# SeanChenxy/TDRN

Measured on AMD Instinct MI355X. Metric: frames/sec/GPU @320x320 dualrefinedet_vggbn; box Linf vs CPU ref, higher is better.
Workload: dtype bf16; 1 GPU; dualrefinedet_vggbn 320x320 multihead, bf16, batch 32 per GPU, forward + Detect(top_k 200, conf 0.01, nms 0.45), synthetic VOC-shaped frames + synthetic weights; global_batch=32, parallelism=frame-sharded x1, no per-frame collective, launch=eager, resident_batches=4, steps_in_flight=2

## Files before the change

include/tdrn_hip.h:

```cpp
#ifndef TDRN_HIP_H
#define TDRN_HIP_H

#include <stddef.h>
#include <stdint.h>

#ifdef __cplusplus
extern "C" {
#endif

#define TDRN_API __attribute__((visibility("default")))

#define TDRN_OK 0
#define TDRN_E_ARG (-1)
#define TDRN_E_SHAPE (-2)
#define TDRN_E_WORKSPACE (-3)
#define TDRN_E_UNSUPPORTED (-4)
#define TDRN_E_PARAM (-5)
#define TDRN_E_STATE (-6)
#define TDRN_E_VALUE (-7)
#define TDRN_E_DEVICE (-8)

TDRN_API const char *tdrn_version(void);
TDRN_API const char *tdrn_error_string(int code);

// ... 233 lines not shown
                         int32_t *counts_out, void *workspace, size_t workspace_bytes,
                         void *stream);
TDRN_API int tdrn_detect_dev_scale(const float *loc, const float *conf, const float *priors,
                                   const float *arm_loc, const float *scale_dev, int B, int P, int C,
                                   int top_k, float conf_thresh, double nms_thresh, float *out,
                                   int32_t *counts_out, void *workspace, size_t workspace_bytes,
                                   void *stream);

TDRN_API int tdrn_preprocess(const uint8_t *frames, int B, int H0, int W0, int S, const float mean_bgr[3],
                             int to_rgb, float *out, void *stream);
TDRN_API int tdrn_preprocess_u8(const uint8_t *frames, int B, int H0, int W0, int S, int to_rgb, uint8_t *out, void *stream);

typedef enum {
    TDRN_DRN_VGGBN = 0,
    TDRN_DRN_MOBILENET = 1,
    TDRN_SSD4SCALE_MOBILE = 2,
    TDRN_REFINEDET_VGG = 3,
    TDRN_SSD4SCALE_VGG = 4
} tdrn_model;

typedef struct {
    int model;
    int size;
    int num_classes;
    int c7_channel;
    int def_groups;
    int bn;
    int multihead;
    int deform;
    int test_phase;
    int dtype;
    int use_refine;
    int plan_flags;
    int reserved[4];
} tdrn_net_config;

#define TDRN_PLAN_NO_FUSE_FIRST 1
#define TDRN_PLAN_NO_LATE_SIDE  2
#define TDRN_PLAN_ONE_STREAM    4
#define TDRN_PLAN_NO_DEFORM_TS  8
#define TDRN_PLAN_CHAIN         16
#define TDRN_PLAN_NO_CONV_PP    32
#define TDRN_PLAN_NO_PP_SK      64
#define TDRN_PLAN_NO_CONV_PATCH 128
#define TDRN_PLAN_DWPW          512
#define TDRN_PLAN_NO_PW1X1      1024
#define TDRN_PLAN_NO_DW_SLIDE   2048
#define TDRN_PLAN_DW_SLIDE_ALL  4096
#define TDRN_PLAN_NO_CONV_WS    8192
#define TDRN_PLAN_NO_YGEMM_V2  16384
#define TDRN_PLAN_NO_HEAD3X3   32768
#define TDRN_PLAN_TS_ONE_RANGE  65536
#define TDRN_PLAN_NO_PATCH_TAIL 131072
#define TDRN_PLAN_FAULT_HANDOFF 256

typedef struct tdrn_net tdrn_net;

TDRN_API int tdrn_net_create(const tdrn_net_config *cfg, tdrn_net **out);
TDRN_API void tdrn_net_destroy(tdrn_net *net);

TDRN_API int tdrn_net_param_count(const tdrn_net *net);
TDRN_API int tdrn_net_param_info(const tdrn_net *net, int index, const char **name,
                                 int64_t shape[4], int *ndim);
TDRN_API int tdrn_net_set_param(tdrn_net *net, const char *name, const float *data_host,
                                int64_t numel);

TDRN_API size_t tdrn_net_weight_bytes(const tdrn_net *net);
TDRN_API size_t tdrn_net_workspace_bytes(const tdrn_net *net, int batch);
TDRN_API int tdrn_net_num_priors(const tdrn_net *net);

TDRN_API int tdrn_net_pack_weights(tdrn_net *net, void *weights_dev, size_t weights_bytes,
                                   void *stream);
TDRN_API int tdrn_net_adopt_weights(tdrn_net *net);

typedef struct {
    const float *x;
    int batch;
    float *arm_loc;
    float *odm_loc;
    float *conf;
    float *offsets[4];
    const float *ref_loc[4];
    float *loc_maps[4];
    void *reserved[4];
} tdrn_net_io;
typedef struct {
    const uint8_t *planes;
    float mean[3];
} tdrn_u8_frames;

TDRN_API int tdrn_net_forward(tdrn_net *net, const void *weights_dev, void *workspace,
                              size_t workspace_bytes, const tdrn_net_io *io, void *stream);

TDRN_API int tdrn_net_check(tdrn_net *net, unsigned *detail);

typedef struct {
    char name[48];
    int launches;
    double flops;
    double bytes;
    double ms;
} tdrn_kernel_stat;
TDRN_API int tdrn_net_profile(tdrn_net *net, int enable);
TDRN_API int tdrn_net_kernel_stats(tdrn_net *net, tdrn_kernel_stat *out, int max_entries);
TDRN_API int tdrn_net_op_stats(tdrn_net *net, tdrn_kernel_stat *out, int max_entries);
TDRN_API int tdrn_net_op_timeline(tdrn_net *net, float *start_ms, float *end_ms, int *lane, int max_entries);
// ... 34 lines not shown
```

tdrn_amd/_lib.py:

```python
import ctypes as C
import os

_HERE = os.path.dirname(os.path.abspath(__file__))
LIB_PATH = os.environ.get("TDRN_LIB_PATH") or os.path.join(_HERE, "lib", "libtdrn_hip.so")

F32, BF16, F16 = 0, 1, 2
DTYPES = {"fp32": F32, "f32": F32, "float32": F32, "bf16": BF16, "bfloat16": BF16, "fp16": F16,
          "f16": F16, "float16": F16, "half": F16}
DRN_VGGBN, DRN_MOBILENET, SSD4SCALE_MOBILE, REFINEDET_VGG, SSD4SCALE_VGG = range(5)

E_VALUE = -7


class TdrnError(RuntimeError):
    def __init__(self, code, what=""):
        self.code = code
        super().__init__("%s (tdrn error %d)%s" % (error_string(code), code,
                                                    (": " + what) if what else ""))


class NetConfig(C.Structure):
    _fields_ = [("model", C.c_int), ("size", C.c_int), ("num_classes", C.c_int),
                ("c7_channel", C.c_int), ("def_groups", C.c_int), ("bn", C.c_int),
                ("multihead", C.c_int), ("deform", C.c_int), ("test_phase", C.c_int),
                ("dtype", C.c_int), ("use_refine", C.c_int), ("plan_flags", C.c_int), ("reserved", C.c_int * 4)]


PLAN_NO_FUSE_FIRST, PLAN_NO_LATE_SIDE, PLAN_ONE_STREAM, PLAN_NO_DEFORM_TS, PLAN_CHAIN = 1, 2, 4, 8, 16
PLAN_NO_CONV_PP, PLAN_NO_PP_SK, PLAN_NO_CONV_PATCH, PLAN_FAULT_HANDOFF, PLAN_DWPW, PLAN_NO_PW1X1 = 32, 64, 128, 256, 512, 1024
PLAN_NO_DW_SLIDE, PLAN_DW_SLIDE_ALL, PLAN_NO_CONV_WS, PLAN_NO_YGEMM_V2, PLAN_NO_HEAD3X3, PLAN_TS_ONE_RANGE = 2048, 4096, 8192, 16384, 32768, 65536
PLAN_NO_PATCH_TAIL = 131072
E_DEVICE = -8


class NetIO(C.Structure):
    _fields_ = [("x", C.c_void_p), ("batch", C.c_int), ("arm_loc", C.c_void_p),
                ("odm_loc", C.c_void_p), ("conf", C.c_void_p), ("offsets", C.c_void_p * 4),
                ("ref_loc", C.c_void_p * 4), ("loc_maps", C.c_void_p * 4),
                ("reserved", C.c_void_p * 4)]


class KernelStat(C.Structure):
    _fields_ = [("name", C.c_char * 48), ("launches", C.c_int), ("flops", C.c_double),
                ("bytes", C.c_double), ("ms", C.c_double)]


class U8FramesABI(C.Structure):
    _fields_ = [("planes", C.c_void_p), ("mean", C.c_float * 3)]


class OpInfo(C.Structure):
    _fields_ = [("kind", C.c_int), ("in_", C.c_int), ("out", C.c_int), ("res", C.c_int), ("pool", C.c_int), ("off", C.c_int),
                ("y", C.c_int), ("k", C.c_int), ("stride", C.c_int), ("pad", C.c_int), ("dil", C.c_int), ("relu", C.c_int),
                ("ceil_mode", C.c_int), ("splitk", C.c_int), ("groups", C.c_int), ("out_kind", C.c_int), ("level", C.c_int),
                ("n_branches", C.c_int), ("k2", C.c_int), ("pad2", C.c_int), ("off_c0", C.c_int * 2), ("y_tap_major", C.c_int),
                ("fused_first", C.c_int), ("fused_dw", C.c_int), ("w", C.c_char * 48), ("b", C.c_char * 48), ("bn", C.c_char * 48), ("w2", C.c_char * 48),
                ("b2", C.c_char * 48), ("y_groups", C.c_int)]


class AugmentParams(C.Structure):
    _fields_ = [("brightness", C.c_float), ("contrast_pre", C.c_float), ("contrast_post", C.c_float), ("saturation", C.c_float),
                ("hue", C.c_float), ("perm", C.c_int32 * 3), ("canvas_w", C.c_int32), ("canvas_h", C.c_int32),
                ("img_x", C.c_int32), ("img_y", C.c_int32), ("crop_x0", C.c_int32), ("crop_y0", C.c_int32),
                ("crop_x1", C.c_int32), ("crop_y1", C.c_int32), ("cropped", C.c_int32), ("mirror", C.c_int32),
                ("kept", C.c_int32), ("status", C.c_int32)]


class AugmentImage(C.Structure):
    _fields_ = [("data", C.c_void_p), ("h", C.c_int32), ("w", C.c_int32)]


class AugmentPairParams(C.Structure):
    _fields_ = [("base", AugmentParams), ("shift_x", C.c_double), ("shift_y", C.c_double), ("trans_x", C.c_int32),
                ("trans_y", C.c_int32), ("attempts", C.c_int32), ("reserved", C.c_int32)]


class SgdTensor(C.Structure):
    _fields_ = [("param", C.c_void_p), ("grad", C.c_void_p), ("momentum_buf", C.c_void_p), ("numel", C.c_int64),
                ("group", C.c_int32), ("reserved", C.c_int32)]


SGD_ZERO_GRADS, SGD_CHUNK, SGD_TENSORS_PER_LAUNCH = 1, 4096, 96
AUGMENT_MAX_TRUTHS, AUGMENT_MAX_SIZE = 512, 2048
AUGMENT_CROP_FALLBACK, AUGMENT_TAPE_EXHAUSTED, AUGMENT_TRANS_FALLBACK = 1, 2, 4
# ... 159 lines not shown
```

tdrn_amd/csrc/conv3x3_patch.hip:

```cpp
#include <cstdio>
#include <cstdlib>
#include <type_traits>

#include "kernels.h"
#include "mfma_prims.h"

#ifndef TDRN_PATCH_PRIO
#define TDRN_PATCH_PRIO 4
#endif
#ifndef TDRN_PATCH_ABLATE
#define TDRN_PATCH_ABLATE 0
#endif

namespace tdrn {

struct PatchParams {
    const char *in, *w, *zero;
    const float *bias;
    char *out, *out_pool;
    int B, H, W, Cin, Cout, Cs, Ktot;
    int relu;
    int tw, lgtw;
    int tiles_x, tiles_per_img;
    int m_tiles, n_tiles, items;
    int M;
    int tail_split;
    const float *fx, *fw, *fb;
    int fS, fCout;
    int ablate;
#ifdef TDRN_PATCH_STAMP
    unsigned *stamps;
#endif
#ifdef TDRN_PATCH_WGTIME
    unsigned long long *wgt;
#endif
};

#ifdef TDRN_PATCH_STAMP
#define STAMP_DECL unsigned long long st_t = __builtin_amdgcn_s_memtime(); unsigned st_acc[8] = {0, 0, 0, 0, 0, 0, 0, 0};
#define STAMP(k) do { const unsigned long long t_ = __builtin_amdgcn_s_memtime(); st_acc[k] += (unsigned)(t_ - st_t); st_t = t_; } while (0)
#define STAMP_FLUSH do { if (lane == 0) for (int k_ = 0; k_ < 8; ++k_) p.stamps[((size_t)blockIdx.x * 12 + wave) * 8 + k_] = st_acc[k_]; } while (0)
#else
#define STAMP_DECL
#define STAMP(k) do { } while (0)
#define STAMP_FLUSH do { } while (0)
#endif

namespace {

#ifndef TDRN_PATCH_RING
#define TDRN_PATCH_RING 3
#endif
constexpr int kRing = TDRN_PATCH_RING;
constexpr int kPatchSlots = kRing == 4 ? 43 : 44;
constexpr int kSlotsPerLoader = (kPatchSlots + 3) / 4;

}

template <typename DT, int BN, int TW, bool FUSE = false>
__global__ __launch_bounds__(768) void conv3x3_patch_kernel(const PatchParams p)
{
    static_assert(!FUSE || (BN == 64 && TW == 32 && sizeof(DT) == 2), "fused first conv: 16-bit, 64 couts, 8x32 tiles");
    constexpr bool FLAT = TW == 0;
    constexpr int LGTW = TW == 32 ? 5 : 4;
    constexpr int TPX = FUSE ? 512 : 256;
    constexpr int TH = TW ? TPX / TW : 0;
    constexpr int PXG = TPX / 64;
    constexpr int CG = 8 / PXG;
    constexpr int ES = elem_traits<DT>::bytes;
    constexpr int P16 = elem_traits<DT>::per16;
    constexpr int CK = 128 / ES;
    constexpr int BNH = BN / CG;
    constexpr int WC = BNH / 32;
    constexpr int WBYTES = BN * 128;
    constexpr int WL = BN / 32;
    constexpr int RING = BN == 128 ? kRing : 3;
    constexpr int SROWS = (ES == 2 ? 16 : 8) / ((RING == 4 && BN == 128) ? 2 : 1);
    constexpr int SSTRIDE = BNH * ES + 16;
    constexpr int NPB = FUSE ? 1 : 2;
    constexpr int PSLOTS = FUSE ? ((TH + 2) * (TW + 2) + 7) / 8 : kPatchSlots;
    constexpr int PBYTES = PSLOTS * 1024;
    constexpr int OFF_W = NPB * PBYTES;
    constexpr int OFF_S = OFF_W + RING * WBYTES;
    constexpr int OFF_B = OFF_S + 8 * SROWS * SSTRIDE;
    constexpr int RAWR = TH + 4, RAWC = 36;
    constexpr int RAWN = 3 * RAWR * RAWC;
    constexpr int RAWP = (RAWN + 63) / 64, RAWJ = (RAWP + 3) / 4;
    constexpr int FTILES = ((TH + 2) * (TW + 2) + 31) / 32, FTJ = (FTILES + 3) / 4;
    constexpr int RAWB = ((RAWN + 63) / 64) * 256;
    constexpr int OFF_R = OFF_B + 1024;
    constexpr int LDS = FUSE ? OFF_R + 2 * RAWB + 256 : OFF_B + 1024;
    static_assert(LDS <= 160 * 1024, "LDS budget");
    __shared__ __attribute__((aligned(16))) char smem[LDS];

    const int lane = threadIdx.x & 63;
    const int wave = __builtin_amdgcn_readfirstlane(threadIdx.x >> 6);
    const int nchunks = p.Cin / CK;
#ifdef TDRN_PATCH_WGTIME
    if (threadIdx.x == 0) p.wgt[2 * blockIdx.x] = __builtin_amdgcn_s_memrealtime();
#endif

    const XcdItems xi = xcd_items(p.items);
    const int slot = xi.slot, istride = xi.istride;
    int avail = p.items - xi.xcd * xi.per_xcd;
    avail = avail < xi.per_xcd ? avail : xi.per_xcd;
    int n_full = avail > slot ? (avail - slot + istride - 1) / istride : 0;
    const int item0 = xi.item0();
    [[maybe_unused]] int n_tail = 0, tail_enc = 0;
    constexpr bool TAILOK = BN == 128 && sizeof(DT) == 2 && !FUSE;
    if constexpr (TAILOK) {
        if (p.tail_split && avail > 0) {
            const int full = avail / istride, rem = avail - full * istride;
            if (full > 0 && rem > 0 && 2 * rem <= istride) {
                n_full = full;
                if (slot < 2 * rem) {
                    n_tail = 1;
                    tail_enc = 2 * (xi.xcd * xi.per_xcd + full * istride) + slot;
                }
            }
        }
    }
    const int n_it = n_full + n_tail;
    const int n_steps = n_it * nchunks * 9;
    auto item_mt = [&](int it) { return (it < n_full ? item0 + it * istride : tail_enc >> 1) / p.n_tiles; };
    auto item_c0 = [&](int it) {
        const int item = it < n_full ? item0 + it * istride : tail_enc >> 1;
        return (item % p.n_tiles) * BN + (it < n_full ? 0 : (tail_enc & 1) * 64);
    };
    const int RS = TW ? TW + 2 : p.W;

    if (wave >= 8) {
        if (TDRN_PATCH_PRIO == 4) __builtin_amdgcn_s_setprio(2);
        if (TDRN_PATCH_PRIO == 5) __builtin_amdgcn_s_setprio(3);
        const int lw = wave - 8;
        const int lrow = lane >> 3, pc = lane & 7;
        unsigned poff[kSlotsPerLoader];
        int pyx[kSlotsPerLoader];
// ... 164 lines not shown
                char *dst = smem + OFF_W + wslot * WBYTES;
#pragma unroll
                for (int k = 0; k < WL; ++k)
                    if (!TAILOK || k < np) lds_dma16_ptr(wfixed ? p.w + (woff[k] & 0xffffu) : wbase + wk + woff[k], dst + (lw + 4 * k) * 1024);
            }
            ++ws;
            wslot = wslot == RING - 1 ? 0 : wslot + 1;
            wk += (unsigned)(p.Cin * ES);
            if (++w_tap == 9) {
                w_tap = 0;
                if (++w_cc == nchunks) {
                    w_cc = 0;
                    ++w_it;
                    if (w_it < n_it) weight_item();
                }
                wk = (unsigned)(w_cc * 128);
            }
            return np;
        };
        auto load_patch = [&](int j, unsigned ccoff, char *dstbuf) {
            if (!live || lw + 4 * j >= kPatchSlots || FUSE) return;
            const unsigned o = poff[j];
            lds_dma16_ptr(o == 0xFFFFFFFFu ? p.zero : (pfixed ? p.in + (o & 0xfffffu) : p.in + (size_t)o + ccoff), dstbuf + (lw + 4 * j) * 1024);
        };
        int p_it = 0, p_cc = 0, pbuf = 0;
        auto next_patch_chunk = [&]() {
            if (NPB == 2) pbuf ^= 1;
            if (++p_cc == nchunks) {
                p_cc = 0;
                ++p_it;
            }
        };

        if constexpr (FUSE) {
            if (n_it > 0) load_raw(item0, 0);
            asm volatile("s_waitcnt vmcnt(0) lgkmcnt(0)" ::: "memory");
            __builtin_amdgcn_s_barrier();
            if (n_it > 0) {
                int b_;
                tile_origin(item0, b_, f_y0, f_x0);
#pragma unroll
                for (int q = 0; q < FTJ; ++q)
                    if (lw + 4 * q < FTILES) first_conv_tile(lw + 4 * q, 0, smem);
            }
        }
        if (n_it > 0) {
            weight_item();
            if constexpr (!FUSE) {
                patch_table(item_mt(0));
#pragma unroll
                for (int j = 0; j < kSlotsPerLoader; ++j) load_patch(j, 0u, smem);
            }
#pragma unroll
            for (int k = 0; k < RING - 1; ++k)
                if (k < n_steps) load_weights();
            next_patch_chunk();
            if (lw == 0 && live)
                lds_dma16_ptr(lane < (n_full > 0 ? BN : 64) / 4 ? (const char *)(p.bias + item_c0(0)) + lane * 16 : p.zero, smem + OFF_B);
        }
        asm volatile("s_waitcnt vmcnt(0) lgkmcnt(0)" ::: "memory");
        __builtin_amdgcn_s_barrier();

        int tap = 0, c_it = 0, c_cc = 0, carried = 0;
        STAMP_DECL
        const int last_piece = lw + 4 * (kSlotsPerLoader - 1) < kPatchSlots ? 1 : 0;
        for (int g = 0; g < n_steps; ++g) {
            int issued = 0;
            if (ws < n_steps) issued = load_weights();
            if constexpr (FUSE) {
                if (tap == 0 && c_it + 1 < n_it) issued += load_raw(item0 + (c_it + 1) * istride, (c_it + 1) & 1);
            } else if (p_it < n_it && tap < 6) {
                char *dstbuf = smem + pbuf * PBYTES;
                const unsigned ccoff = (unsigned)(p_cc * 128);
                switch (tap) {
                    case 0:
                        patch_table(item_mt(p_it));
                        load_patch(0, ccoff, dstbuf); load_patch(1, ccoff, dstbuf); issued += 2; break;
                    case 1: load_patch(2, ccoff, dstbuf); load_patch(3, ccoff, dstbuf); issued += 2; break;
                    case 2: load_patch(4, ccoff, dstbuf); load_patch(5, ccoff, dstbuf); issued += 2; break;
                    case 3: load_patch(6, ccoff, dstbuf); load_patch(7, ccoff, dstbuf); issued += 2; break;
                    case 4: load_patch(8, ccoff, dstbuf); load_patch(9, ccoff, dstbuf); issued += 2; break;
                    default: load_patch(10, ccoff, dstbuf); issued += last_piece; break;
                }
            }
            if (lw == 0 && c_cc == nchunks - 1 && tap == 6 && c_it + 1 < n_it) {
                if (live) lds_dma16_ptr(lane < (c_it + 1 < n_full ? BN : 64) / 4 ? (const char *)(p.bias + item_c0(c_it + 1)) + lane * 16 : p.zero, smem + OFF_B);
                issued += 1;
            }
            STAMP(0);
            wait_vmcnt(live ? issued + (RING == 4 ? carried : 0) : 0);
            if constexpr (FUSE) asm volatile("s_waitcnt lgkmcnt(0)" ::: "memory");
            STAMP(1);
            carried = issued;
            __builtin_amdgcn_s_barrier();
            STAMP(2);
            if (++tap == 9) {
                tap = 0;
                next_patch_chunk();
                if (++c_cc == nchunks) {
                    if constexpr (FUSE) {
                        if (c_it + 1 < n_it) {
                            int b_;
                            tile_origin(item0 + (c_it + 1) * istride, b_, f_y0, f_x0);
#pragma unroll
                            for (int q = 0; q < FTJ; ++q)
                                if (lw + 4 * q < FTILES) first_conv_tile(lw + 4 * q, (c_it + 1) & 1, smem);
                            asm volatile("s_waitcnt lgkmcnt(0)" ::: "memory");
                            __builtin_amdgcn_s_barrier();
                        }
                    }
                    c_cc = 0;
                    ++c_it;
                }
            }
        }
        STAMP_FLUSH;
        return;
    }

    const int r32 = lane & 31, hh = lane >> 5;
    const int cw = wave % PXG;
    const int chalf = wave / PXG;
    char *stg = smem + OFF_S + wave * SROWS * SSTRIDE;
    f32x16 acc[WC][2];

    int base_i[2];
    unsigned tapmask[2] = {0x1FFu, 0x1FFu};
    unsigned need_mask = 0;
#pragma unroll
    for (int pt = 0; pt < 2; ++pt) {
        const int i = cw * 64 + pt * 32 + r32;
        base_i[pt] = TW ? (i >> LGTW) * RS + (i & (TW - 1)) : i;
    }
    const int wsw = (r32 >> 1) & 7;
    constexpr int CPR = BNH * ES / 16;
    constexpr int RPI = 64 / CPR;
    const int my_ch = lane % CPR, my_row = lane / CPR;
    constexpr bool compute = !(TDRN_PATCH_ABLATE & 2);

    int cur_mt = -1, n0 = 0;
    long long tile_pix0 = 0;
    int tile_row0 = 0, tile_x0 = 0;
    auto setup_item = [&](int it) {
        const int mt = item_mt(it);
        n0 = item_c0(it);
        if (mt == cur_mt) return;
// ... 219 lines not shown
    int psw[2] = {(base_i[0] >> 1) & 7, (base_i[1] >> 1) & 7};
    auto load_frags = [&](auto wcn_tag, u32x4 *wf, u32x4 *pf, int kk) {
        constexpr int WCN = decltype(wcn_tag)::value;
        if (!compute) return;
        const int lc = 2 * kk + hh;
#pragma unroll
        for (int ci = 0; ci < WCN; ++ci) wf[ci] = *(const u32x4 *)(wsb + (chalf * (32 * WCN) + ci * 32 + r32) * 128 + ((lc ^ wsw) << 4));
#pragma unroll
        for (int pt = 0; pt < 2; ++pt) pf[pt] = *(const u32x4 *)(psb + prow[pt] * 128 + ((lc ^ psw[pt]) << 4));
    };
    auto mma_frags = [&](auto wcn_tag, const u32x4 *wf, u32x4 *pf, unsigned m0, unsigned m1) {
        constexpr int WCN = decltype(wcn_tag)::value;
        if (!compute) return;
        if constexpr (FLAT) {
#pragma unroll
            for (int j = 0; j < 4; ++j) {
                pf[0][j] &= m0;
                pf[1][j] &= m1;
            }
        }
#pragma unroll
        for (int ci = 0; ci < WCN; ++ci)
#pragma unroll
            for (int pt = 0; pt < 2; ++pt) Mma32<DT>::run(wf[ci], pf[pt], acc[ci][pt]);
    };
    auto init_acc = [&](auto wcn_tag) {
        constexpr int WCN = decltype(wcn_tag)::value;
        const char *bsrc = smem + OFF_B;
#pragma unroll
        for (int ci = 0; ci < WCN; ++ci)
#pragma unroll
            for (int g = 0; g < 4; ++g) {
                const f32x4 bv = *(const f32x4 *)(bsrc + (chalf * (32 * WCN) + ci * 32 + 8 * g + 4 * hh) * 4);
#pragma unroll
                for (int pt = 0; pt < 2; ++pt)
#pragma unroll
                    for (int j = 0; j < 4; ++j) acc[ci][pt][4 * g + j] = bv[j];
            }
    };

    if constexpr (FUSE) __builtin_amdgcn_s_barrier();
    __builtin_amdgcn_s_barrier();
    if (TDRN_PATCH_PRIO == 2 && wave >= 4) __builtin_amdgcn_s_setprio(1);
    if (TDRN_PATCH_PRIO == 3) __builtin_amdgcn_s_setprio(1);
    typedef std::integral_constant<int, WC> full_t;
    typedef std::integral_constant<int, 1> half_t;
    if (n_it > 0) {
        setup_item(0);
        init_acc(full_t{});
        load_frags(full_t{}, wfA, pfA, 0);
    }
    int it = 0, cc = 0, tap = 0, tq = 0, delta = 0, wslot = 0, pbuf = 0;
    STAMP_DECL
    auto step = [&](auto wcn) {
        unsigned m0 = 0xFFFFFFFFu, m1 = 0xFFFFFFFFu;
        if constexpr (FLAT) {
            m0 = ((tapmask[0] >> tap) & 1u) ? 0xFFFFFFFFu : 0u;
            m1 = ((tapmask[1] >> tap) & 1u) ? 0xFFFFFFFFu : 0u;
        }
        if (TDRN_PATCH_PRIO == 0) __builtin_amdgcn_s_setprio(1);
        load_frags(wcn, wfB, pfB, 1);
        __builtin_amdgcn_sched_barrier(0);
        mma_frags(wcn, wfA, pfA, m0, m1);
        __builtin_amdgcn_sched_barrier(0);
        load_frags(wcn, wfA, pfA, 2);
        __builtin_amdgcn_sched_barrier(0);
        mma_frags(wcn, wfB, pfB, m0, m1);
        __builtin_amdgcn_sched_barrier(0);
        load_frags(wcn, wfB, pfB, 3);
        __builtin_amdgcn_sched_barrier(0);
        mma_frags(wcn, wfA, pfA, m0, m1);
        if (TDRN_PATCH_PRIO == 0) __builtin_amdgcn_s_setprio(0);
        __builtin_amdgcn_s_waitcnt(0xC07F);
        STAMP(0);
        __builtin_amdgcn_s_barrier();
        STAMP(1);
        const bool item_done = tap == 8 && cc == nchunks - 1;
        wslot = wslot == RING - 1 ? 0 : wslot + 1;
        ++tap;
        if (++tq == 3) {
            tq = 0;
            delta += RS;
        }
        if (tap == 9) {
            tap = 0; tq = 0; delta = 0;
            pbuf ^= 1;
            if (++cc == nchunks) cc = 0;
        }
        wsb = smem + OFF_W + wslot * WBYTES;
        psb = smem + (NPB == 2 ? pbuf : 0) * PBYTES;
#pragma unroll
        for (int pt = 0; pt < 2; ++pt) {
            prow[pt] = base_i[pt] + delta + tq;
            psw[pt] = (prow[pt] >> 1) & 7;
        }
        if (!(FUSE && item_done)) load_frags(wcn, wfA, pfA, 0);
        __builtin_amdgcn_sched_barrier(0);
        if (TDRN_PATCH_PRIO == 0) __builtin_amdgcn_s_setprio(1);
        mma_frags(wcn, wfB, pfB, m0, m1);
        if (TDRN_PATCH_PRIO == 0) __builtin_amdgcn_s_setprio(0);
        STAMP(2);
        if (item_done) {
            epilogue(wcn);
            ++it;
            if (it < n_it) {
                setup_item(it);
                if (TAILOK && it >= n_full) {
                    init_acc(half_t{});
                    load_frags(half_t{}, wfA, pfA, 0);
                } else {
                    init_acc(full_t{});
                }
                if constexpr (FUSE) {
                    __builtin_amdgcn_s_barrier();
                    load_frags(wcn, wfA, pfA, 0);
                }
            }
            STAMP(3);
        }
    };
    const int n_steps_full = n_full * nchunks * 9;
#pragma unroll 1
    for (int g = 0; g < n_steps_full; ++g) step(full_t{});
    if constexpr (TAILOK) {
#pragma unroll 1
        for (int g = n_steps_full; g < n_steps; ++g) step(half_t{});
    }
    STAMP_FLUSH;
#ifdef TDRN_PATCH_WGTIME
    if (threadIdx.x == 0) p.wgt[2 * blockIdx.x + 1] = __builtin_amdgcn_s_memrealtime();
#endif
}

bool patch_takes(const ConvArgs &a, bool pooled)
{
    if ((a.kdisable & KOFF_CONV_PATCH) || a.fuse_x8 || !conv3x3_input_fits(a)) return false;
    const int mode = conv3x3_tile_mode(a, kPatchSlots);
    if (pooled && (mode < 0 || (a.H & 1) || (a.W & 1))) return false;
    if (a.fuse_x && (a.dtype == TDRN_F32 || mode != 32 || a.Npad != 64 || a.H % 16)) return false;
    return mode != 0;
}

template <typename DT, int BN> static int launch_patch_cfg(const PatchParams &p_in, hipStream_t s)
{
    PatchParams p = p_in;
    const int grid = persistent_grid(p.items);
#ifdef TDRN_PATCH_WGTIME
    static unsigned long long *wgt = nullptr;
    static long calls = 0, want = -1;
    if (!wgt) TDRN_HIP_TRY(hipMalloc((void **)&wgt, 256 * 2 * sizeof(unsigned long long)));
    if (want < 0) { const char *e = getenv("TDRN_WGTIME_CALL"); want = e ? atol(e) : 2000; }
    p.wgt = wgt;
    const bool report = calls >= want && calls < want + 18;
    ++calls;
    if (report) TDRN_HIP_TRY(hipMemsetAsync(wgt, 0, 256 * 2 * sizeof(unsigned long long), s));
    struct Report {
        bool on; hipStream_t s; int grid; const PatchParams &p; unsigned long long *d;
        ~Report() {
            if (!on) return;
            (void)hipStreamSynchronize(s);
            unsigned long long h[512];
            (void)hipMemcpy(h, d, sizeof(h), hipMemcpyDeviceToHost);
            unsigned long long t0 = ~0ull, t1 = 0;
            int n = 0;
            for (int i = 0; i < grid; ++i) if (h[2 * i]) { t0 = h[2 * i] < t0 ? h[2 * i] : t0; t1 = h[2 * i + 1] > t1 ? h[2 * i + 1] : t1; ++n; }
            double late = 0, busy = 0, worst = 0, e_min = 1e18; int n5 = 0, n20 = 0;
            for (int i = 0; i < grid; ++i) if (h[2 * i]) {
                const double d0 = (h[2 * i] - t0) * 0.01, b = (h[2 * i + 1] - h[2 * i]) * 0.01, e = (h[2 * i + 1] - t0) * 0.01;
                late += d0; busy += b; worst = d0 > worst ? d0 : worst; e_min = e < e_min ? e : e_min; n5 += d0 > 5; n20 += d0 > 20;
            }
            fprintf(stderr, "wgtime %dx%d Cin %d Cout %d items %d grid %d: span %.1f us, workgroup busy mean %.1f us, first end at %.1f us; start later than the first: mean %.1f us, max %.1f us, > 5 us: %d, > 20 us: %d of %d\n",
                    p.H, p.W, p.Cin, p.Cout, p.items, grid, (t1 - t0) * 0.01, busy / n, e_min, late / n, worst, n5, n20, n);
        }
    } rep{report, s, grid, p, wgt};
#endif
    if constexpr (BN == 64 && sizeof(DT) == 2) {
        if (p.fx) {
            hipLaunchKernelGGL((conv3x3_patch_kernel<DT, 64, 32, true>), dim3(grid), dim3(768), 0, s, p);
            return hip_status(hipGetLastError());
        }
    }
    if (p.fx) return TDRN_E_UNSUPPORTED;
    if (p.tw == 0) hipLaunchKernelGGL((conv3x3_patch_kernel<DT, BN, 0>), dim3(grid), dim3(768), 0, s, p);
    else if (p.tw == 32) hipLaunchKernelGGL((conv3x3_patch_kernel<DT, BN, 32>), dim3(grid), dim3(768), 0, s, p);
    else hipLaunchKernelGGL((conv3x3_patch_kernel<DT, BN, 16>), dim3(grid), dim3(768), 0, s, p);
    return hip_status(hipGetLastError());
}

int launch_conv3x3_patch(const ConvArgs &a, void *out_pool, hipStream_t s)
{
    if (!patch_takes(a, out_pool != nullptr)) return TDRN_E_UNSUPPORTED;
    const int mode = conv3x3_tile_mode(a, kPatchSlots);
    PatchParams p;
    p.in = (const char *)a.in; p.w = (const char *)a.w; p.zero = (const char *)a.zero_page; p.bias = a.bias;
    p.out = (char *)a.out; p.out_pool = (char *)out_pool;
    p.B = a.B; p.H = a.H; p.W = a.W; p.Cin = a.Cin; p.Cout = a.Cout; p.Cs = (int)a.o_cs; p.Ktot = 9 * a.Cin;
    p.relu = a.relu;
    p.tw = mode > 0 ? mode : 0;
    p.lgtw = mode == 32 ? 5 : (mode == 16 ? 4 : 0);
    p.M = a.B * a.H * a.W;
    conv_tiles(a.B, a.H, a.W, p.tw, a.fuse_x ? 512 : 256, p.tiles_x, p.tiles_per_img, p.m_tiles);
    int BN = a.Npad % 128 == 0 ? 128 : 64;
    if (BN == 128 && p.m_tiles * (a.Npad / 128) < 160) BN = 64;
    p.n_tiles = a.Npad / BN;
    p.items = p.m_tiles * p.n_tiles;
    static int ablate = -1;
    if (ablate < 0) ablate = dev_ablate_env("TDRN_CONV_ABLATE");
    p.ablate = ablate;
    p.fx = a.fuse_x; p.fw = a.fuse_w; p.fb = a.fuse_b; p.fS = a.H; p.fCout = a.fuse_cout;
    p.tail_split = !(a.kdisable & KOFF_PATCH_TAIL);
    if (p.items <= 0) return TDRN_OK;
#ifdef TDRN_PATCH_STAMP
    static unsigned *stamps = nullptr;
    if (!stamps) TDRN_HIP_TRY(hipMalloc((void **)&stamps, 256 * 12 * 8 * sizeof(unsigned)));
    TDRN_HIP_TRY(hipMemsetAsync(stamps, 0, 256 * 12 * 8 * sizeof(unsigned), s));
    p.stamps = stamps;
    struct Report {
        const PatchParams &p; hipStream_t s; int BN, nchunks;
        ~Report()
        {
            static unsigned host[256 * 12 * 8];
            (void)hipStreamSynchronize(s);
            (void)hipMemcpy(host, p.stamps, sizeof(host), hipMemcpyDeviceToHost);
            double c[4] = {0, 0, 0, 0}, l[3] = {0, 0, 0};
            int nc = 0, nl = 0;
            for (int b = 0; b < 256; ++b)
                for (int w = 0; w < 12; ++w) {
                    const unsigned *v = host + (b * 12 + w) * 8;
                    if (v[0] + v[1] + v[2] == 0) continue;
                    if (w < 8) { for (int k = 0; k < 4; ++k) c[k] += v[k]; ++nc; }
                    else { for (int k = 0; k < 3; ++k) l[k] += v[k]; ++nl; }
                }
            if (!nc || !nl) return;
            const double steps = (double)((p.items + 255) / 256) * nchunks * 9;
            fprintf(stderr, "patch_stamp H%d W%d Cin%d Cout%d BN%d tw%d items%d steps/CU~%.0f | consumer cyc/wave: slices0-2 %.0f barrier %.0f slice3 %.0f epilogue %.0f"
                            " | loader cyc/wave: issue %.0f vmcnt %.0f barrier %.0f\n",
                    p.H, p.W, p.Cin, p.Cout, BN, p.tw, p.items, steps, c[0] / nc, c[1] / nc, c[2] / nc, c[3] / nc, l[0] / nl, l[1] / nl, l[2] / nl);
        }
    } report{p, s, BN, (int)(p.Cin * dtype_bytes(a.dtype) / 128)};
#endif
#define LP(DT)                                                    \
    return BN == 128 ? launch_patch_cfg<DT, 128>(p, s) : launch_patch_cfg<DT, 64>(p, s)
    switch (a.dtype) {
        case TDRN_F32: LP(float);
        case TDRN_BF16: LP(bf16_t);
        case TDRN_F16: LP(f16_t);
    }
#undef LP
    return TDRN_E_ARG;
}

}
```

tdrn_amd/csrc/kernels.h:

```cpp
#pragma once
#include <cmath>

#include "common.h"

namespace tdrn {

constexpr size_t kZeroPageBytes = 256;

int allow_big_lds(const void *kernel);

enum KernelOff {
    KOFF_CONV_PP = 1,
    KOFF_PP_SK = 2,
    KOFF_CONV_PATCH = 4,
    KOFF_PW1X1 = 8,
    KOFF_DW_SLIDE = 16,
    KOFF_DW_STRIP_SMALL = 32,
    KOFF_CONV_WS = 64,
    KOFF_YGEMM_V2 = 128,
    KOFF_HEAD3X3 = 256,
    KOFF_TS_RANGES = 512,
    KOFF_PATCH_TAIL = 1024,
};

struct ConvArgs {
    const void *in = nullptr, *w = nullptr, *res = nullptr, *zero_page = nullptr;
    const float *bias = nullptr;
    void *out = nullptr;
    int B = 0, H = 0, W = 0, Cin = 0;
    int Ho = 0, Wo = 0, Cout = 0, Npad = 0;
    int kh = 1, kw = 1, stride = 1, pad = 0, dil = 1;
    int relu = 0, out_f32 = 0, phases = 1;
    int splitk = 1;
    void *partial = nullptr;
    long long o_bs = 0, o_rs = 0, o_cs = 0, o_base = 0, o_pr = 0, o_pc = 0;
    int dtype = TDRN_BF16;
    const float *fuse_x = nullptr, *fuse_w = nullptr, *fuse_b = nullptr;
    int fuse_cout = 0;
    const unsigned char *fuse_x8 = nullptr;
    float fuse_mean[3] = {0.f, 0.f, 0.f};
    void *sk_ws = nullptr;
    bool sk_flags_zero = false;
    int kdisable = 0;
    unsigned *status = nullptr;
    int fault_handoff = 0;
};
enum ConvKernel { CONV_IGEMM, CONV_PATCH, CONV_PP, CONV_WS, CONV_HEAD3X3, CONV_PW1X1, CONV_NONE };
ConvKernel conv_route(const ConvArgs &a, bool pooled);
const char *conv_kernel_name(ConvKernel k);
int launch_conv(const ConvArgs &a, hipStream_t s, void *out_pool = nullptr);
int conv_splitk_choice(const ConvArgs &a);
int launch_conv_igemm(const ConvArgs &a, hipStream_t s);
int igemm_splitk_choice(const ConvArgs &a);
size_t conv_splitk_bytes(const ConvArgs &a, int splits);
struct ChainLayer { ConvArgs a; int dep[2] = {-1, -1}; };
int conv_chain_supported(const ConvArgs &a);
int conv_chain_max_layers();
size_t conv_chain_ctr_bytes();
int launch_conv_chain(const ChainLayer *layers, int n, unsigned *ctr, hipStream_t s, unsigned *status = nullptr);
bool head3x3_takes(const ConvArgs &a, bool pooled);
int launch_head3x3(const ConvArgs &a, hipStream_t s);
inline int conv3x3_tile_mode(const ConvArgs &a, int slots)
{
    if (a.kh != 3 || a.kw != 3 || a.stride != 1 || a.pad != 1 || a.dil != 1 || a.phases != 1 || a.out_f32 || a.res) return 0;
    if (a.Ho != a.H || a.Wo != a.W || a.Npad % 64) return 0;
    if (a.o_rs != (long long)a.Wo * a.o_cs || a.o_bs != (long long)a.Ho * a.Wo * a.o_cs || a.o_base) return 0;
    if (a.W % 32 == 0 && a.H % 8 == 0) return 32;
    if (a.W % 16 == 0 && a.H % 16 == 0) return 16;
    return 2 * a.W + 2 + 256 <= slots * 8 ? -1 : 0;
}
inline bool conv3x3_input_fits(const ConvArgs &a) { return a.fuse_x || (long long)a.B * a.H * a.W * a.Cin * dtype_bytes(a.dtype) < (1ll << 32); }
bool patch_takes(const ConvArgs &a, bool pooled);
int launch_conv3x3_patch(const ConvArgs &a, void *out_pool, hipStream_t s);
bool pp_takes_geometry(const ConvArgs &a);
bool pp_takes(const ConvArgs &a, bool pooled);
// ... 186 lines not shown
```

tdrn_amd/csrc/net_plan.hip:

```cpp
#include <algorithm>
#include <cstdlib>

#include "net_plan.h"

namespace tdrn {

int Plan::T(int C, int H, int W, bool f32)
{
    Tensor t;
    t.C = C; t.H = H; t.W = W; t.f32 = f32;
    t.Cpad = f32 ? C : (int)align_up((size_t)C, kChanPad);
    t.off = ws_per_sample;
    ws_per_sample += align_up((size_t)t.Cpad * H * W * (f32 ? 4 : es), 256);
    tensors.push_back(t);
    return (int)tensors.size() - 1;
}
void Plan::P_(const std::string &name, std::vector<int64_t> shape)
{
    param_index[name] = params.size();
    params.push_back(ParamSpec{name, std::move(shape)});
}
void Plan::bn_params(const std::string &bn, int C)
{
    P_(bn + ".weight", {C}); P_(bn + ".bias", {C}); P_(bn + ".running_mean", {C}); P_(bn + ".running_var", {C});
// ... 574 lines not shown
        Op &d = ops[i];
        Op &c = ops[i + 1];
        if (d.kind != OP_DW || c.kind != OP_CONV || c.in != d.out || c.k != 1 || c.stride != 1 || c.pad != 0 || c.phases != 1 || c.res >= 0 ||
            c.out_kind != OUT_TENSOR || c.splitk != 1 || c.lane != d.lane || c.pool_t >= 0 || c.chain >= 0) continue;
        if (readers_of(d.out) != 1) continue;
        const Tensor &ti = tensors[d.in];
        DwPwArgs a;
        a.B = 1; a.H = ti.H; a.W = ti.W; a.Cin = c.Cin; a.Cout = c.Cout; a.Npad = c.Npad; a.Cs = tensors[c.out].Cpad;
        a.stride = d.stride; a.dtype = cfg.dtype;
        if (ti.Cpad != c.Cin || !dwpw_supported(a)) continue;
        d.fused_dw = 1; c.fused_dw = 1;
        d.stat = ST_DWPW;
        d.flops += c.flops;
        d.bytes = (double)ti.H * ti.W * ti.Cpad * es + (double)ti.H * ti.W * tensors[c.out].Cpad * es;
        c.flops = 0; c.bytes = 0;
    }
}

void Plan::plan_workspace_tail()
{
    ws_fixed = 0;
    pp_sk_planned = false;
    for (const Op &o : ops) {
        if (o.kind != OP_CONV || o.stat != ST_CONV3 || o.lane != 0) continue;
        ConvArgs a = conv_question(o, 0);
        a.kdisable = 0;
        pp_sk_planned = pp_sk_planned || pp_takes_geometry(a);
    }
    if (pp_sk_planned || !chain_ops.empty()) ws_fixed = kTailCtl + (pp_sk_planned ? align_up(conv_pp_sk_bytes(), 256) : 1024);
}

void Plan::mark_shared_tensors()
{
    tensor_lane.assign(tensors.size(), 0);
    tensor_shared.assign(tensors.size(), 0);
    for (const Op &o : ops) {
        if (o.out >= 0) tensor_lane[o.out] = o.lane;
        if (o.pool_t >= 0) tensor_lane[o.pool_t] = o.lane;
    }
    for (const Op &o : ops)
        for (int t : {o.in, o.res, o.off_t})
            if (t >= 0 && tensor_lane[t] != o.lane) tensor_shared[t] = 1;
}

int Plan::build()
{
    es = dtype_bytes(cfg.dtype);
    static const struct { int plan_flag, koff; } kSwitches[] = {
        {TDRN_PLAN_NO_CONV_PP, KOFF_CONV_PP},       {TDRN_PLAN_NO_PP_SK, KOFF_PP_SK},
        {TDRN_PLAN_NO_CONV_PATCH, KOFF_CONV_PATCH}, {TDRN_PLAN_NO_PW1X1, KOFF_PW1X1},
        {TDRN_PLAN_NO_DW_SLIDE, KOFF_DW_SLIDE},     {TDRN_PLAN_DW_SLIDE_ALL, KOFF_DW_STRIP_SMALL},
        {TDRN_PLAN_NO_CONV_WS, KOFF_CONV_WS},       {TDRN_PLAN_NO_YGEMM_V2, KOFF_YGEMM_V2},
        {TDRN_PLAN_NO_HEAD3X3, KOFF_HEAD3X3},       {TDRN_PLAN_TS_ONE_RANGE, KOFF_TS_RANGES},
        {TDRN_PLAN_NO_PATCH_TAIL, KOFF_PATCH_TAIL},
    };
    kdisable = 0;
    for (const auto &sw : kSwitches)
        if (cfg.plan_flags & sw.plan_flag) kdisable |= sw.koff;
    fault_handoff = (cfg.plan_flags & TDRN_PLAN_FAULT_HANDOFF) ? 1 : 0;
    late_side = !(cfg.plan_flags & TDRN_PLAN_NO_LATE_SIDE);
    use_lanes = !(cfg.plan_flags & TDRN_PLAN_ONE_STREAM);
    if (cfg.size < 128 || cfg.size > 1280 || cfg.size % 64 != 0) return TDRN_E_ARG;
    if (cfg.num_classes < 2 || cfg.num_classes > 21 * 4) return TDRN_E_ARG;
    if (cfg.dtype < 0 || cfg.dtype > 2) return TDRN_E_ARG;
    if (cfg.def_groups < 1) return TDRN_E_ARG;
    int rc;
    switch (cfg.model) {
        case TDRN_DRN_VGGBN: rc = build_drn(false); break;
        case TDRN_DRN_MOBILENET: rc = build_drn(true); break;
        case TDRN_SSD4SCALE_MOBILE: rc = build_ssd4scale(true); break;
        case TDRN_SSD4SCALE_VGG: rc = build_ssd4scale(false); break;
        case TDRN_REFINEDET_VGG: rc = build_refinedet_vgg(); break;
        default: return TDRN_E_UNSUPPORTED;
    }
    if (rc != TDRN_OK) return rc;
    if (plan_error != TDRN_OK) return plan_error;
    alias_u8_input();
    hoist_l2norm_to_side_lanes();
    plan_fuse_first();
    plan_splitk();
    plan_chain();
    place_splitk_slabs();
    plan_dwpw();
    plan_workspace_tail();
    y_tap_major = true;
    for (const Op &d : ops)
        if (d.kind == OP_DEFORM && d.y_t >= 0 && !ygemm_supported(d.Cin, d.y_cols, cfg.dtype)) y_tap_major = false;
    mark_shared_tensors();
    return TDRN_OK;
}

}
```

Baseline: 11960 frames/s.

## Pair 3x3 patch conv taps per barrier to halve workgroup synchronisations

Adds a PAIR variant of the persistent 3x3 patch conv kernel for 16-bit, BN=64, flat-tile layers. Consumer waves run two taps per barrier (groups of 2,2,2,2,1 per chunk), and loader waves issue two weight slices per group on a 4-deep weight ring. The patch pieces are spread across five barrier groups instead of nine. It also drops the unused staging LDS region for 16-bit non-fused kernels and removes the ring-4 compile option. The aim is to cut barrier and wait overhead in the producer/consumer pipeline, at the cost of more LDS for weights and less slack between load and use.

```diff
diff --git a/include/tdrn_hip.h b/include/tdrn_hip.h
--- a/include/tdrn_hip.h
+++ b/include/tdrn_hip.h
@@ -309,6 +309,7 @@
 #define TDRN_PLAN_NO_HEAD3X3   32768
 #define TDRN_PLAN_TS_ONE_RANGE  65536
 #define TDRN_PLAN_NO_PATCH_TAIL 131072
+#define TDRN_PLAN_NO_PATCH_PAIR 262144
 #define TDRN_PLAN_FAULT_HANDOFF 256
 
 typedef struct tdrn_net tdrn_net;
diff --git a/tdrn_amd/_lib.py b/tdrn_amd/_lib.py
--- a/tdrn_amd/_lib.py
+++ b/tdrn_amd/_lib.py
@@ -29,7 +29,7 @@
 PLAN_NO_FUSE_FIRST, PLAN_NO_LATE_SIDE, PLAN_ONE_STREAM, PLAN_NO_DEFORM_TS, PLAN_CHAIN = 1, 2, 4, 8, 16
 PLAN_NO_CONV_PP, PLAN_NO_PP_SK, PLAN_NO_CONV_PATCH, PLAN_FAULT_HANDOFF, PLAN_DWPW, PLAN_NO_PW1X1 = 32, 64, 128, 256, 512, 1024
 PLAN_NO_DW_SLIDE, PLAN_DW_SLIDE_ALL, PLAN_NO_CONV_WS, PLAN_NO_YGEMM_V2, PLAN_NO_HEAD3X3, PLAN_TS_ONE_RANGE = 2048, 4096, 8192, 16384, 32768, 65536
-PLAN_NO_PATCH_TAIL = 131072
+PLAN_NO_PATCH_TAIL, PLAN_NO_PATCH_PAIR = 131072, 262144
 E_DEVICE = -8
 
 
diff --git a/tdrn_amd/csrc/conv3x3_patch.hip b/tdrn_amd/csrc/conv3x3_patch.hip
--- a/tdrn_amd/csrc/conv3x3_patch.hip
+++ b/tdrn_amd/csrc/conv3x3_patch.hip
@@ -48,19 +48,22 @@
 
 namespace {
 
-#ifndef TDRN_PATCH_RING
-#define TDRN_PATCH_RING 3
-#endif
-constexpr int kRing = TDRN_PATCH_RING;
-constexpr int kPatchSlots = kRing == 4 ? 43 : 44;
+constexpr int kPatchSlots = 44;
 constexpr int kSlotsPerLoader = (kPatchSlots + 3) / 4;
 
+__device__ __forceinline__ int opaque_s(int v)
+{
+    asm volatile("" : "+s"(v));
+    return v;
 }
 
-template <typename DT, int BN, int TW, bool FUSE = false>
+}
+
+template <typename DT, int BN, int TW, bool FUSE = false, bool PAIR = false>
 __global__ __launch_bounds__(768) void conv3x3_patch_kernel(const PatchParams p)
 {
     static_assert(!FUSE || (BN == 64 && TW == 32 && sizeof(DT) == 2), "fused first conv: 16-bit, 64 couts, 8x32 tiles");
+    static_assert(!PAIR || (sizeof(DT) == 2 && !FUSE), "barrier groups: 16-bit, not the fused first conv");
     constexpr bool FLAT = TW == 0;
     constexpr int LGTW = TW == 32 ? 5 : 4;
     constexpr int TPX = FUSE ? 512 : 256;
@@ -74,15 +77,17 @@
     constexpr int WC = BNH / 32;
     constexpr int WBYTES = BN * 128;
     constexpr int WL = BN / 32;
-    constexpr int RING = BN == 128 ? kRing : 3;
-    constexpr int SROWS = (ES == 2 ? 16 : 8) / ((RING == 4 && BN == 128) ? 2 : 1);
+    constexpr bool SLIM = sizeof(DT) == 2 && !FUSE;
+    constexpr int NSLOT = SLIM ? 4 : 3;
+    constexpr int RING = PAIR ? 4 : 3;
+    constexpr int SROWS = ES == 2 ? 16 : 8;
     constexpr int SSTRIDE = BNH * ES + 16;
     constexpr int NPB = FUSE ? 1 : 2;
     constexpr int PSLOTS = FUSE ? ((TH + 2) * (TW + 2) + 7) / 8 : kPatchSlots;
     constexpr int PBYTES = PSLOTS * 1024;
     constexpr int OFF_W = NPB * PBYTES;
-    constexpr int OFF_S = OFF_W + RING * WBYTES;
-    constexpr int OFF_B = OFF_S + 8 * SROWS * SSTRIDE;
+    constexpr int OFF_S = OFF_W + NSLOT * WBYTES;
+    constexpr int OFF_B = OFF_S + (SLIM ? 0 : 8 * SROWS * SSTRIDE);
     constexpr int RAWR = TH + 4, RAWC = 36;
     constexpr int RAWN = 3 * RAWR * RAWC;
     constexpr int RAWP = (RAWN + 63) / 64, RAWJ = (RAWP + 3) / 4;
@@ -353,7 +358,7 @@
                 for (int j = 0; j < kSlotsPerLoader; ++j) load_patch(j, 0u, smem);
             }
 #pragma unroll
-            for (int k = 0; k < RING - 1; ++k)
+            for (int k = 0; k < 2; ++k)
                 if (k < n_steps) load_weights();
             next_patch_chunk();
             if (lw == 0 && live)
@@ -362,9 +367,49 @@
         asm volatile("s_waitcnt vmcnt(0) lgkmcnt(0)" ::: "memory");
         __builtin_amdgcn_s_barrier();
 
-        int tap = 0, c_it = 0, c_cc = 0, carried = 0;
+        int tap = 0, c_it = 0, c_cc = 0;
         STAMP_DECL
         const int last_piece = lw + 4 * (kSlotsPerLoader - 1) < kPatchSlots ? 1 : 0;
+        if constexpr (PAIR) {
+            static_assert(kSlotsPerLoader == 11, "patch pieces per barrier group: 3, 3, 3, 2");
+            const int n_groups = n_it * nchunks * 5;
+            for (int g = 0; g < n_groups; ++g) {
+                if (ws < n_steps) load_weights();
+                if (tap != 4 && ws < n_steps) load_weights();
+                int later = 0;
+                if (p_it < n_it && tap < 4) {
+                    char *dstbuf = smem + pbuf * PBYTES;
+                    const unsigned ccoff = (unsigned)(p_cc * 128);
+                    switch (tap) {
+                        case 0:
+                            patch_table(item_mt(p_it));
+                            load_patch(0, ccoff, dstbuf); load_patch(1, ccoff, dstbuf); load_patch(2, ccoff, dstbuf); later += 3; break;
+                        case 1: load_patch(3, ccoff, dstbuf); load_patch(4, ccoff, dstbuf); load_patch(5, ccoff, dstbuf); later += 3; break;
+                        case 2: load_patch(6, ccoff, dstbuf); load_patch(7, ccoff, dstbuf); load_patch(8, ccoff, dstbuf); later += 3; break;
+                        default: load_patch(9, ccoff, dstbuf); load_patch(10, ccoff, dstbuf); later += 1 + last_piece; break;
+                    }
+                }
+                if (lw == 0 && c_cc == nchunks - 1 && tap == 3 && c_it + 1 < n_it) {
+                    if (live) lds_dma16_ptr(lane < (c_it + 1 < n_full ? BN : 64) / 4 ? (const char *)(p.bias + item_c0(c_it + 1)) + lane * 16 : p.zero, smem + OFF_B);
+                    later += 1;
+                }
+                STAMP(0);
+                wait_vmcnt(live ? later : 0);
+                STAMP(1);
+                __builtin_amdgcn_s_barrier();
+                STAMP(2);
+                if (++tap == 5) {
+                    tap = 0;
+                    next_patch_chunk();
+                    if (++c_cc == nchunks) {
+                        c_cc = 0;
+                        ++c_it;
+                    }
+                }
+            }
+            STAMP_FLUSH;
+            return;
+        }
         for (int g = 0; g < n_steps; ++g) {
             int issued = 0;
             if (ws < n_steps) issued = load_weights();
@@ -389,10 +434,9 @@
                 issued += 1;
             }
             STAMP(0);
-            wait_vmcnt(live ? issued + (RING == 4 ? carried : 0) : 0);
+            wait_vmcnt(live ? issued : 0);
             if constexpr (FUSE) asm volatile("s_waitcnt lgkmcnt(0)" ::: "memory");
             STAMP(1);
-            carried = issued;
             __builtin_amdgcn_s_barrier();
             STAMP(2);
             if (++tap == 9) {
@@ -718,7 +762,12 @@
     }
     int it = 0, cc = 0, tap = 0, tq = 0, delta = 0, wslot = 0, pbuf = 0;
     STAMP_DECL
-    auto step = [&](auto wcn) {
+    typedef std::integral_constant<int, 0> any_t;
+    typedef std::integral_constant<int, 1> open_t;
+    typedef std::integral_constant<int, 2> close_t;
+    typedef std::integral_constant<int, 3> last_t;
+    auto step = [&](auto wcn, auto pos) {
+        constexpr int POS = decltype(pos)::value;
         unsigned m0 = 0xFFFFFFFFu, m1 = 0xFFFFFFFFu;
         if constexpr (FLAT) {
             m0 = ((tapmask[0] >> tap) & 1u) ? 0xFFFFFFFFu : 0u;
@@ -737,19 +786,27 @@
         __builtin_amdgcn_sched_barrier(0);
         mma_frags(wcn, wfA, pfA, m0, m1);
         if (TDRN_PATCH_PRIO == 0) __builtin_amdgcn_s_setprio(0);
-        __builtin_amdgcn_s_waitcnt(0xC07F);
-        STAMP(0);
-        __builtin_amdgcn_s_barrier();
-        STAMP(1);
-        const bool item_done = tap == 8 && cc == nchunks - 1;
+        if constexpr (POS == 1) {
+            __builtin_amdgcn_sched_barrier(0);
+        } else {
+            __builtin_amdgcn_s_waitcnt(0xC07F);
+            STAMP(0);
+            __builtin_amdgcn_s_barrier();
+            STAMP(1);
+        }
+        const bool item_done = POS == 0 ? (tap == 8 && cc == nchunks - 1) : (POS == 3 && cc == nchunks - 1);
         wslot = wslot == RING - 1 ? 0 : wslot + 1;
         ++tap;
         if (++tq == 3) {
             tq = 0;
             delta += RS;
         }
-        if (tap == 9) {
-            tap = 0; tq = 0; delta = 0;
+        if (POS == 0 ? tap == 9 : POS == 3) {
+            if constexpr (POS == 3) {
+                tap = opaque_s(0); tq = opaque_s(0); delta = opaque_s(0);
+            } else {
+                tap = 0; tq = 0; delta = 0;
+            }
             pbuf ^= 1;
             if (++cc == nchunks) cc = 0;
         }
@@ -765,8 +822,8 @@
         if (TDRN_PATCH_PRIO == 0) __builtin_amdgcn_s_setprio(1);
         mma_frags(wcn, wfB, pfB, m0, m1);
         if (TDRN_PATCH_PRIO == 0) __builtin_amdgcn_s_setprio(0);
-        STAMP(2);
-        if (item_done) {
+        if constexpr (POS != 1) STAMP(2);
+        if constexpr (POS == 0 || POS == 3) if (item_done) {
             epilogue(wcn);
             ++it;
             if (it < n_it) {
@@ -785,12 +842,31 @@
             STAMP(3);
         }
     };
-    const int n_steps_full = n_full * nchunks * 9;
+    if constexpr (PAIR) {
+        auto chunk = [&](auto wcn) {
+#pragma unroll
+            for (int k = 0; k < 4; ++k) {
+                step(wcn, open_t{});
+                step(wcn, close_t{});
+            }
+            step(wcn, last_t{});
+        };
+        const int n_chunks_full = n_full * nchunks;
 #pragma unroll 1
-    for (int g = 0; g < n_steps_full; ++g) step(full_t{});
-    if constexpr (TAILOK) {
+        for (int c = 0; c < n_chunks_full; ++c) chunk(full_t{});
+        if constexpr (TAILOK) {
+            const int n_chunks_half = n_tail * nchunks;
 #pragma unroll 1
-        for (int g = n_steps_full; g < n_steps; ++g) step(half_t{});
+            for (int c = 0; c < n_chunks_half; ++c) chunk(half_t{});
+        }
+    } else {
+        const int n_steps_full = n_full * nchunks * 9;
+#pragma unroll 1
+        for (int g = 0; g < n_steps_full; ++g) step(full_t{}, any_t{});
+        if constexpr (TAILOK) {
+#pragma unroll 1
+            for (int g = n_steps_full; g < n_steps; ++g) step(half_t{}, any_t{});
+        }
     }
     STAMP_FLUSH;
 #ifdef TDRN_PATCH_WGTIME
@@ -807,7 +883,7 @@
     return mode != 0;
 }
 
-template <typename DT, int BN> static int launch_patch_cfg(const PatchParams &p_in, hipStream_t s)
+template <typename DT, int BN> static int launch_patch_cfg(const PatchParams &p_in, bool pair, hipStream_t s)
 {
     PatchParams p = p_in;
     const int grid = persistent_grid(p.items);
@@ -847,6 +923,12 @@
         }
     }
     if (p.fx) return TDRN_E_UNSUPPORTED;
+    if constexpr (sizeof(DT) == 2 && BN == 64) {
+        if (pair && p.tw == 0) {
+            hipLaunchKernelGGL((conv3x3_patch_kernel<DT, BN, 0, false, true>), dim3(grid), dim3(768), 0, s, p);
+            return hip_status(hipGetLastError());
+        }
+    }
     if (p.tw == 0) hipLaunchKernelGGL((conv3x3_patch_kernel<DT, BN, 0>), dim3(grid), dim3(768), 0, s, p);
     else if (p.tw == 32) hipLaunchKernelGGL((conv3x3_patch_kernel<DT, BN, 32>), dim3(grid), dim3(768), 0, s, p);
     else hipLaunchKernelGGL((conv3x3_patch_kernel<DT, BN, 16>), dim3(grid), dim3(768), 0, s, p);
@@ -875,6 +957,7 @@
     p.ablate = ablate;
     p.fx = a.fuse_x; p.fw = a.fuse_w; p.fb = a.fuse_b; p.fS = a.H; p.fCout = a.fuse_cout;
     p.tail_split = !(a.kdisable & KOFF_PATCH_TAIL);
+    const bool pair = !(a.kdisable & KOFF_PATCH_PAIR) && a.dtype != TDRN_F32 && !a.fuse_x && p.tw == 0 && BN == 64;
     if (p.items <= 0) return TDRN_OK;
 #ifdef TDRN_PATCH_STAMP
     static unsigned *stamps = nullptr;
@@ -882,7 +965,7 @@
     TDRN_HIP_TRY(hipMemsetAsync(stamps, 0, 256 * 12 * 8 * sizeof(unsigned), s));
     p.stamps = stamps;
     struct Report {
-        const PatchParams &p; hipStream_t s; int BN, nchunks;
+        const PatchParams &p; hipStream_t s; int BN, nchunks; bool pair;
         ~Report()
         {
             static unsigned host[256 * 12 * 8];
@@ -899,14 +982,14 @@
                 }
             if (!nc || !nl) return;
             const double steps = (double)((p.items + 255) / 256) * nchunks * 9;
-            fprintf(stderr, "patch_stamp H%d W%d Cin%d Cout%d BN%d tw%d items%d steps/CU~%.0f | consumer cyc/wave: slices0-2 %.0f barrier %.0f slice3 %.0f epilogue %.0f"
+            fprintf(stderr, "patch_stamp H%d W%d Cin%d Cout%d BN%d tw%d %s items%d steps/CU~%.0f | consumer cyc/wave: slices0-2 %.0f barrier %.0f slice3 %.0f epilogue %.0f"
                             " | loader cyc/wave: issue %.0f vmcnt %.0f barrier %.0f\n",
-                    p.H, p.W, p.Cin, p.Cout, BN, p.tw, p.items, steps, c[0] / nc, c[1] / nc, c[2] / nc, c[3] / nc, l[0] / nl, l[1] / nl, l[2] / nl);
-        }
-    } report{p, s, BN, (int)(p.Cin * dtype_bytes(a.dtype) / 128)};
+                    p.H, p.W, p.Cin, p.Cout, BN, p.tw, pair ? "groups" : "taps", p.items, steps, c[0] / nc, c[1] / nc, c[2] / nc, c[3] / nc, l[0] / nl, l[1] / nl, l[2] / nl);
+        }
+    } report{p, s, BN, (int)(p.Cin * dtype_bytes(a.dtype) / 128), pair};
 #endif
 #define LP(DT)                                                    \
-    return BN == 128 ? launch_patch_cfg<DT, 128>(p, s) : launch_patch_cfg<DT, 64>(p, s)
+    return BN == 128 ? launch_patch_cfg<DT, 128>(p, pair, s) : launch_patch_cfg<DT, 64>(p, pair, s)
     switch (a.dtype) {
         case TDRN_F32: LP(float);
         case TDRN_BF16: LP(bf16_t);
diff --git a/tdrn_amd/csrc/kernels.h b/tdrn_amd/csrc/kernels.h
--- a/tdrn_amd/csrc/kernels.h
+++ b/tdrn_amd/csrc/kernels.h
@@ -21,6 +21,7 @@
     KOFF_HEAD3X3 = 256,
     KOFF_TS_RANGES = 512,
     KOFF_PATCH_TAIL = 1024,
+    KOFF_PATCH_PAIR = 2048,
 };
 
 struct ConvArgs {
diff --git a/tdrn_amd/csrc/net_plan.hip b/tdrn_amd/csrc/net_plan.hip
--- a/tdrn_amd/csrc/net_plan.hip
+++ b/tdrn_amd/csrc/net_plan.hip
@@ -650,7 +650,7 @@
         {TDRN_PLAN_NO_DW_SLIDE, KOFF_DW_SLIDE},     {TDRN_PLAN_DW_SLIDE_ALL, KOFF_DW_STRIP_SMALL},
         {TDRN_PLAN_NO_CONV_WS, KOFF_CONV_WS},       {TDRN_PLAN_NO_YGEMM_V2, KOFF_YGEMM_V2},
         {TDRN_PLAN_NO_HEAD3X3, KOFF_HEAD3X3},       {TDRN_PLAN_TS_ONE_RANGE, KOFF_TS_RANGES},
-        {TDRN_PLAN_NO_PATCH_TAIL, KOFF_PATCH_TAIL},
+        {TDRN_PLAN_NO_PATCH_TAIL, KOFF_PATCH_TAIL}, {TDRN_PLAN_NO_PATCH_PAIR, KOFF_PATCH_PAIR},
     };
     kdisable = 0;
     for (const auto &sw : kSwitches)
```

After: 11990 frames/s, median of 6. Within noise of the previous version (+0.3%).
